# EPFL-VILAB/MultiMAE

Hardware: AMD Instinct MI355X
Metric: pre-train images/sec (whole node), ViT-B RGB+D+S 224^2 98-vis-tok (higher is better)
Workload: dtype bf16 (fp32_output_adapters: fp16 storage); 1 GPU; BASELINE.json configs[2]: ViT-B, RGB+depth+semseg, 224^2, Dirichlet alpha=1.0, 98 visible tokens, 4 cross-attention decoders (dim 256, depth 2), semseg adapter (fp32_output_adapters) with fp16 STORAGE (activations / saved tensors / gradients of the adapter as IEEE half in HBM: every matmul input carries the 11-bit significand TF32 gave the reference on A100; gradients stored times a power of two f; per_gpu_batch=256, global_batch=256, parallelism=dp1

## Files before the change

### multimae_amd/csrc/losses.hip

```cpp
#include <math.h>
#include <type_traits>
#include "common.h"

namespace {

constexpr int LSPLIT = 8;

__device__ __forceinline__ void block_sum2(float& a, float& b) {
    __shared__ float ra[4], rb[4];
    a = wave_sum(a); b = wave_sum(b);
    const int w = threadIdx.x >> 6;
    if ((threadIdx.x & 63) == 0) { ra[w] = a; rb[w] = b; }
    __syncthreads();
    if (threadIdx.x == 0) { a = (ra[0] + ra[1]) + (ra[2] + ra[3]); b = (rb[0] + rb[1]) + (rb[2] + rb[3]); }
    __syncthreads();
}

__global__ void __launch_bounds__(256) pixel_loss_fwd_kernel(const float* __restrict__ pred, const float* __restrict__ target,
                                                             const long long* __restrict__ mask, int kind, int norm_pix, int C, int H,
                                                             int W, int P, float* __restrict__ stats, float* __restrict__ partial) {
    const int b = blockIdx.y, nh = H / P, nw = W / P, np = nh * nw;
    const int lane = threadIdx.x & 63, w = threadIdx.x >> 6;
    const int npix = P * P, nval = npix * C;
    float acc = 0.f;
// ... 4 lines not shown
        if (norm_pix) {
            float s = 0.f;
            for (int e = lane; e < nval; e += 64) {
                const int c = e / npix, ij = e % npix;
                s += target[(((long long)b * C + c) * H + py * P + ij / P) * W + px * P + ij % P];
            }
            mu = wave_sum(s) / (float)nval;
            float q = 0.f;
            for (int e = lane; e < nval; e += 64) {
                const int c = e / npix, ij = e % npix;
                const float d = target[(((long long)b * C + c) * H + py * P + ij / P) * W + px * P + ij % P] - mu;
                q += d * d;
            }
            const float var = wave_sum(q) / (float)(nval - 1);
            rs = 1.0f / sqrtf(var + 1e-6f);
            if (lane == 0) { stats[((long long)b * np + p) * 2] = mu; stats[((long long)b * np + p) * 2 + 1] = rs; }
        }
        float s = 0.f;
        for (int e = lane; e < nval; e += 64) {
            const int c = e / npix, ij = e % npix;
            const long long a = (((long long)b * C + c) * H + py * P + ij / P) * W + px * P + ij % P;
            const float t = (target[a] - mu) * rs;
            const float d = pred[a] - t;
            s += kind == 0 ? d * d : fabsf(d);
        }
        s = wave_sum(s);
        if (lane == 0) acc += s;
    }
    float dummy = 0.f;
    block_sum2(acc, dummy);
    if (threadIdx.x == 0) partial[(long long)b * LSPLIT + blockIdx.x] = acc / (float)C;
}

__global__ void __launch_bounds__(256) loss_finalize_kernel(const float* __restrict__ partial, const long long* __restrict__ mask, int B,
                                                            int np, int pix_per_patch, float* __restrict__ per_sample,
                                                            float* __restrict__ loss) {
    float tot = 0.f, nvalid = 0.f;
    for (int b = threadIdx.x; b < B; b += 256) {
        float s = 0.f;
        for (int i = 0; i < LSPLIT; ++i) s += partial[(long long)b * LSPLIT + i];
        int cnt = 0;
        const long long* mrow = mask + (long long)b * np;
        int p = 0;
        if ((((uintptr_t)mrow) & 15) == 0) {
            typedef __attribute__((ext_vector_type(2))) long long ll2;
            const ll2* m2 = reinterpret_cast<const ll2*>(mrow);
            const int n2 = np >> 1;
            int q = 0;
            for (; q + 4 <= n2; q += 4) {
                const ll2 a0 = m2[q], a1 = m2[q + 1], a2 = m2[q + 2], a3 = m2[q + 3];
                cnt += (a0[0] != 0) + (a0[1] != 0) + (a1[0] != 0) + (a1[1] != 0) + (a2[0] != 0) + (a2[1] != 0) + (a3[0] != 0) + (a3[1] != 0);
            }
            for (; q < n2; ++q) { const ll2 a = m2[q]; cnt += (a[0] != 0) + (a[1] != 0); }
            p = n2 * 2;
        }
        for (; p < np; ++p) cnt += mrow[p] != 0;
        const float c = (float)cnt * (float)pix_per_patch;
        per_sample[b * 2] = s; per_sample[b * 2 + 1] = c;
        if (cnt > 0) { tot += s / c; nvalid += 1.f; }
    }
    block_sum2(tot, nvalid);
    if (threadIdx.x == 0) { loss[0] = nvalid > 0.f ? tot / nvalid : 0.f; loss[1] = nvalid; }
}

__global__ void pixel_loss_bwd_kernel(const float* __restrict__ pred, const float* __restrict__ target, const long long* __restrict__ mask,
                                      int kind, int norm_pix, int C, int H, int W, int P, const float* __restrict__ stats,
                                      const float* __restrict__ per_sample, const float* __restrict__ loss, const float* __restrict__ upstream,
                                      float* __restrict__ d_pred, long long total) {
    const long long i = (long long)blockIdx.x * blockDim.x + threadIdx.x;
    if (i >= total) return;
    const int x = (int)(i % W); long long r = i / W;
    const int y = (int)(r % H); r /= H;
    const long long b = r / C;
    const int nw = W / P, np = (H / P) * nw, p = (y / P) * nw + x / P;
    float g = 0.f;
    if (mask[b * np + p] != 0) {
        float mu = 0.f, rs = 1.f;
        if (norm_pix) { mu = stats[(b * np + p) * 2]; rs = stats[(b * np + p) * 2 + 1]; }
        const float d = pred[i] - (target[i] - mu) * rs;
        const float wgt = upstream[0] / (loss[1] * per_sample[b * 2 + 1] * (float)C);
        g = wgt * (kind == 0 ? 2.f * d : (d > 0.f ? 1.f : (d < 0.f ? -1.f : 0.f)));
    }
    d_pred[i] = g;
}

__global__ void __launch_bounds__(256) ce_fwd_kernel(const float* __restrict__ logits, const long long* __restrict__ target,
                                                     const long long* __restrict__ mask, int C, int H, int W, int P, float eps,
                                                     float* __restrict__ lse, float* __restrict__ partial) {
    const int b = blockIdx.y, HW = H * W, nw = W / P, np = (H / P) * nw;
    float acc = 0.f;
    for (int px = blockIdx.x * 256 + threadIdx.x; px < HW; px += LSPLIT * 256) {
        const int y = px / W, x = px % W;
        if (mask[(long long)b * np + (y / P) * nw + x / P] == 0) continue;
        const float* l = logits + (long long)b * C * HW + px;
        float mx = l[0], s = 1.f, sx = l[0];
// ... 259 lines not shown
            float v[8];
#pragma unroll
            for (int k = 0; k < 8; ++k) { const int e = e0 + 64 * k; v[k] = e < nval ? prow[e] : -3.0e38f; }
            float gm = fmaxf(fmaxf(fmaxf(v[0], v[1]), fmaxf(v[2], v[3])), fmaxf(fmaxf(v[4], v[5]), fmaxf(v[6], v[7])));
            if (gm > mx) { s *= expf(mx - gm); mx = gm; }
#pragma unroll
            for (int k = 0; k < 8; ++k) {
                const int e = e0 + 64 * k;
                if (e < nval) {
                    s += expf(v[k] - mx);
                    sx += v[k];
                    if ((long long)(slot + (e >> 6) * nslot) == t) lt = v[k];
                }
            }
        }
        for (int o = npix; o < 64; o <<= 1) {
            const float om = __shfl_xor(mx, o, 64), os = __shfl_xor(s, o, 64);
            lt += __shfl_xor(lt, o, 64);
            sx += __shfl_xor(sx, o, 64);
            const float nm = fmaxf(mx, om);
            s = s * expf(mx - nm) + os * expf(om - nm);
            mx = nm;
        }
        const float ls = mx + logf(s);
        if (slot == 0) { lse_pat[row * npix + pix] = ls; }
        const bool tok = t >= 0 && t < C;
        float contrib = slot == 0 && tok ? (eps == 0.f ? ls - lt : (1.f - eps) * (ls - lt) + eps * (ls - sx / (float)C)) : 0.f;
        contrib = wave_sum(contrib);
        if (lane == 0) acc += contrib;
    }
    float dummy = 0.f;
    block_sum2(acc, dummy);
    if (threadIdx.x == 0) partial[(long long)b * LSPLIT + blockIdx.x] = acc;
}

template <typename DT>
__global__ void __launch_bounds__(256) ce_pat_bwd_kernel(const float* __restrict__ pat, const long long* __restrict__ target,
                                                         const long long* __restrict__ mask, int C, int H, int W, int P, float eps,
                                                         const float* __restrict__ lse_pat, const float* __restrict__ per_sample,
                                                         const float* __restrict__ loss, const float* __restrict__ upstream,
                                                         DT* __restrict__ d_pat, long long ld, long long n_rows, float* __restrict__ amax) {
    const int lane = threadIdx.x & 63;
    const long long row = (long long)blockIdx.x * 4 + (threadIdx.x >> 6);
    const int nw = W / P, np = (H / P) * nw, npix = P * P, nval = npix * C;
    const long long b = row / np;
    const int p = (int)(row % np), py = p / nw, px = p % nw;
    const int pix = lane % npix, slot = lane / npix, nslot = 64 / npix;
    float gs = 1.0f;
    if constexpr (std::is_same<DT, h16_t>::value) {
        __shared__ float wred[4];
        const int B = (int)(n_rows / np);
        float wm = 0.f;
        for (int i = threadIdx.x; i < B; i += 256) {
            const float cnt = per_sample[i * 2 + 1];
            if (cnt > 0.f) wm = fmaxf(wm, fabsf(upstream[0] / (loss[1] * cnt)));
        }
        wm = wave_max(wm);
        if (lane == 0) wred[threadIdx.x >> 6] = wm;
        __syncthreads();
        wm = fmaxf(fmaxf(wred[0], wred[1]), fmaxf(wred[2], wred[3]));
        if (blockIdx.x == 0 && threadIdx.x == 0 && amax) *amax = wm;
        gs = h16_grad_scale(&wm);
    }
    if (row >= n_rows) return;
    const bool on = mask[row] != 0;
    DT* drow = d_pat + row * ld;
    if (!on) {
        for (int e = lane; e < (int)ld; e += 64) ActT<DT>::st(drow + e, 0.f);
        return;
    }
    const float wgt = gs * upstream[0] / (loss[1] * per_sample[b * 2 + 1]);
    const float ls = lse_pat[row * npix + pix];
    const long long t = target[((long long)b * H + py * P + pix / P) * W + px * P + pix % P];
    const bool tok = t >= 0 && t < C;
    const float* prow = pat + row * nval;
    float gmax = 0.f;
    for (int e0 = lane; e0 < (int)ld; e0 += 256) {
        float v[4];
#pragma unroll
        for (int k = 0; k < 4; ++k) { const int e = e0 + 64 * k; v[k] = e < nval ? prow[e] : 0.f; }
#pragma unroll
        for (int k = 0; k < 4; ++k) {
            const int e = e0 + 64 * k;
            if (e < (int)ld) {
                const int c = slot + (e >> 6) * nslot;
                float g = 0.f;
                if (e < nval && tok) g = wgt * (expf(v[k] - ls) - (((long long)c == t ? 1.f - eps : 0.f) + eps / (float)C));
                gmax = fmaxf(gmax, fabsf(g));
                ActT<DT>::st(drow + e, g);
            }
        }
    }
    if (!std::is_same<DT, h16_t>::value && amax) note_amax(gmax, amax);
}

__global__ void __launch_bounds__(256) sumsq_stage1(const float* __restrict__ x, long long n, float* __restrict__ ws) {
    float s = 0.f, d = 0.f;
    for (long long i = ((long long)blockIdx.x * 256 + threadIdx.x) * 4; i < n; i += (long long)gridDim.x * 1024) {
        if (i + 4 <= n) { const f32x4 v = ld4(x + i); s += (v[0] * v[0] + v[1] * v[1]) + (v[2] * v[2] + v[3] * v[3]); }
        else for (long long j = i; j < n; ++j) s += x[j] * x[j];
    }
    block_sum2(s, d);
    if (threadIdx.x == 0) ws[blockIdx.x] = s;
}
// ... 126 lines not shown
    long long nb = cdiv64(d->n, 1024);
    if (nb > 8192) nb = 8192;
    const float* bc = d->state + 5;
    const float* gsc = d->state + 2;
    if (d->shadow && d->shadow_dtype == MMAE_BF16)
        hipLaunchKernelGGL((adamw_groups_kernel<uint16_t, HY, TAIL>), dim3((unsigned)nb), dim3(256), 0, st, d->p, d->g, d->m, d->v, (long long)d->n,
                           d->group_map, (int)d->n_groups, hy, d->beta1, d->beta2, d->eps, bc, gsc, (const int*)d->istate, (uint16_t*)d->shadow, n_norm, (const float*)(d->state + 7));
    else
        hipLaunchKernelGGL((adamw_groups_kernel<float, HY, TAIL>), dim3((unsigned)nb), dim3(256), 0, st, d->p, d->g, d->m, d->v, (long long)d->n,
                           d->group_map, (int)d->n_groups, hy, d->beta1, d->beta2, d->eps, bc, gsc, (const int*)d->istate, (float*)d->shadow, n_norm, (const float*)(d->state + 7));
    return mmae_check_launch("adamw_groups");
}

inline bool shadow_ok(const void* shadow, int dtype) {
    if (!shadow) return true;
    return (dtype == MMAE_F32 && (uintptr_t)shadow % 16 == 0) || (dtype == MMAE_BF16 && (uintptr_t)shadow % 8 == 0);
}
#define MMAE_SHADOW_MSG ": shadow must be MMAE_F32 (16-byte aligned) or MMAE_BF16 (8-byte aligned)"

}

extern "C" {

int mmae_masked_pixel_loss_fwd(const float* pred, const float* target, const int64_t* mask, int kind, int norm_pix, int B, int C,
                               int H, int W, int patch, float* stats, float* partial, float* per_sample, float* loss, void* stream) {
    MMAE_REQUIRE(pred && target && mask && partial && per_sample && loss, "pixel_loss_fwd: null pointer");
    MMAE_REQUIRE(!norm_pix || stats, "pixel_loss_fwd: norm_pix needs stats");
    MMAE_REQUIRE(patch > 0 && H % patch == 0 && W % patch == 0 && (kind == 0 || kind == 1), "pixel_loss_fwd: bad geometry");
    hipStream_t st = (hipStream_t)stream;
    hipLaunchKernelGGL(pixel_loss_fwd_kernel, dim3(LSPLIT, B), dim3(256), 0, st, pred, target, (const long long*)mask, kind, norm_pix, C, H,
                       W, patch, stats, partial);
    int rc = mmae_check_launch("pixel_loss_fwd");
    if (rc) return rc;
    hipLaunchKernelGGL(loss_finalize_kernel, dim3(1), dim3(256), 0, st, partial, (const long long*)mask, B, (H / patch) * (W / patch),
                       patch * patch, per_sample, loss);
    return mmae_check_launch("loss_finalize");
}

int mmae_masked_pixel_loss_bwd(const float* pred, const float* target, const int64_t* mask, int kind, int norm_pix, int B, int C,
                               int H, int W, int patch, const float* stats, const float* per_sample, const float* loss,
                               const float* upstream, float* d_pred, void* stream) {
    MMAE_REQUIRE(pred && target && mask && per_sample && loss && upstream && d_pred, "pixel_loss_bwd: null pointer");
    const long long total = (long long)B * C * H * W;
    if (W % 4 == 0 && patch % 4 == 0 && ((uintptr_t)pred % 16 == 0) && ((uintptr_t)target % 16 == 0) && ((uintptr_t)d_pred % 16 == 0))
        hipLaunchKernelGGL(pixel_loss_bwd4_kernel, dim3((unsigned)cdiv64(total / 4, 256)), dim3(256), 0, (hipStream_t)stream, pred, target,
                           (const long long*)mask, kind, norm_pix, C, H, W, patch, stats, per_sample, loss, upstream, d_pred, total / 4);
    else
    hipLaunchKernelGGL(pixel_loss_bwd_kernel, dim3((unsigned)cdiv64(total, 256)), dim3(256), 0, (hipStream_t)stream, pred, target,
                       (const long long*)mask, kind, norm_pix, C, H, W, patch, stats, per_sample, loss, upstream, d_pred, total);
    return mmae_check_launch("pixel_loss_bwd");
}

int mmae_masked_ce_fwd(const float* logits, const int64_t* target, const int64_t* mask, int B, int C, int H, int W, int patch,
                       float label_smoothing, float* lse, float* partial, float* per_sample, float* loss, void* stream) {
    MMAE_REQUIRE(logits && target && mask && lse && partial && per_sample && loss, "ce_fwd: null pointer");
    MMAE_REQUIRE(patch > 0 && H % patch == 0 && W % patch == 0, "ce_fwd: bad geometry");
    hipStream_t st = (hipStream_t)stream;
    MMAE_REQUIRE(label_smoothing >= 0.f && label_smoothing <= 1.f, "ce_fwd: label_smoothing outside [0, 1]");
    hipLaunchKernelGGL(ce_fwd_kernel, dim3(LSPLIT, B), dim3(256), 0, st, logits, (const long long*)target, (const long long*)mask, C, H, W,
                       patch, label_smoothing, lse, partial);
    int rc = mmae_check_launch("ce_fwd");
    if (rc) return rc;
    hipLaunchKernelGGL(loss_finalize_kernel, dim3(1), dim3(256), 0, st, partial, (const long long*)mask, B, (H / patch) * (W / patch),
                       patch * patch, per_sample, loss);
    return mmae_check_launch("loss_finalize");
}

int mmae_masked_ce_bwd(const float* logits, const int64_t* target, const int64_t* mask, int B, int C, int H, int W, int patch,
                       float label_smoothing, const float* lse, const float* per_sample, const float* loss, const float* upstream,
                       float* d_logits, void* stream) {
    MMAE_REQUIRE(logits && target && mask && lse && per_sample && loss && upstream && d_logits, "ce_bwd: null pointer");
    const long long total = (long long)B * C * H * W;
    if (W % 4 == 0 && patch % 4 == 0 && ((uintptr_t)logits % 16 == 0) && ((uintptr_t)lse % 16 == 0) && ((uintptr_t)d_logits % 16 == 0))
        hipLaunchKernelGGL(ce_bwd4_kernel, dim3((unsigned)cdiv64(total / 4, 256)), dim3(256), 0, (hipStream_t)stream, logits,
                           (const long long*)target, (const long long*)mask, C, H, W, patch, label_smoothing, lse, per_sample, loss, upstream, d_logits, total / 4);
    else
    hipLaunchKernelGGL(ce_bwd_kernel, dim3((unsigned)cdiv64(total, 256)), dim3(256), 0, (hipStream_t)stream, logits, (const long long*)target,
                       (const long long*)mask, C, H, W, patch, label_smoothing, lse, per_sample, loss, upstream, d_logits, total);
    return mmae_check_launch("ce_bwd");
}

int mmae_masked_pixel_loss_pat_fwd(const float* pat, const float* target, const int64_t* mask, int kind, int norm_pix, int B, int C, int H,
                                   int W, int patch, float* stats, float* partial, float* per_sample, float* loss, void* stream) {
    MMAE_REQUIRE(pat && target && mask && partial && per_sample && loss, "pixel_loss_pat_fwd: null pointer");
    MMAE_REQUIRE(!norm_pix || stats, "pixel_loss_pat_fwd: norm_pix needs stats");
    MMAE_REQUIRE(patch > 0 && H % patch == 0 && W % patch == 0 && (kind == 0 || kind == 1), "pixel_loss_pat_fwd: bad geometry");
    hipStream_t st = (hipStream_t)stream;
    hipLaunchKernelGGL(pixel_loss_pat_fwd_kernel, dim3(LSPLIT, B), dim3(256), 0, st, pat, target, (const long long*)mask, kind, norm_pix, C, H, W,
                       patch, stats, partial);
    int rc = mmae_check_launch("pixel_loss_pat_fwd");
    if (rc) return rc;
    hipLaunchKernelGGL(loss_finalize_kernel, dim3(1), dim3(256), 0, st, partial, (const long long*)mask, B, (H / patch) * (W / patch),
                       patch * patch, per_sample, loss);
    return mmae_check_launch("loss_finalize");
}

int mmae_masked_pixel_loss_pat_bwd(const float* pat, const float* target, const int64_t* mask, int kind, int norm_pix, int B, int C, int H,
                                   int W, int patch, const float* stats, const float* per_sample, const float* loss, const float* upstream,
                                   void* d_pat, int d_pat_dtype, int64_t ld_pat, float* amax, void* stream) {
    MMAE_REQUIRE(pat && target && mask && per_sample && loss && upstream && d_pat, "pixel_loss_pat_bwd: null pointer");
    MMAE_REQUIRE(patch > 0 && H % patch == 0 && W % patch == 0 && ld_pat >= (int64_t)C * patch * patch, "pixel_loss_pat_bwd: bad geometry");
    MMAE_REQUIRE(!norm_pix || stats, "pixel_loss_pat_bwd: norm_pix needs stats");
    MMAE_REQUIRE(((uintptr_t)pat % 16 == 0) && ((uintptr_t)target % 16 == 0) && ((uintptr_t)d_pat % 16 == 0), "pixel_loss_pat_bwd: unaligned");
    const long long rows = (long long)B * (H / patch) * (W / patch);
    const dim3 grid((unsigned)((rows + 3) / 4));
    if (d_pat_dtype == MMAE_BF16)
        hipLaunchKernelGGL((pixel_loss_pat_bwd_kernel<uint16_t>), grid, dim3(256), 0, (hipStream_t)stream, pat, target, (const long long*)mask, kind,
                           norm_pix, C, H, W, patch, stats, per_sample, loss, upstream, (uint16_t*)d_pat, (long long)ld_pat, rows, amax);
    else
        hipLaunchKernelGGL((pixel_loss_pat_bwd_kernel<float>), grid, dim3(256), 0, (hipStream_t)stream, pat, target, (const long long*)mask, kind,
                           norm_pix, C, H, W, patch, stats, per_sample, loss, upstream, (float*)d_pat, (long long)ld_pat, rows, amax);
    return mmae_check_launch("pixel_loss_pat_bwd");
}

int mmae_masked_ce_pat_fwd(const float* pat, const int64_t* target, const int64_t* mask, int B, int C, int H, int W, int patch,
                           float label_smoothing, float* lse_pat, float* partial, float* per_sample, float* loss, void* stream) {
    MMAE_REQUIRE(pat && target && mask && lse_pat && partial && per_sample && loss, "ce_pat_fwd: null pointer");
    MMAE_REQUIRE(patch > 0 && H % patch == 0 && W % patch == 0, "ce_pat_fwd: bad geometry");
    const int npix = patch * patch;
    if (npix > 64 || (npix & (npix - 1))) { mmae_set_error("ce_pat_fwd: patch_size^2 must be a power of two <= 64"); return MMAE_ESUPPORT; }
    hipStream_t st = (hipStream_t)stream;
    hipLaunchKernelGGL(ce_pat_fwd_kernel, dim3(LSPLIT, B), dim3(256), 0, st, pat, (const long long*)target, (const long long*)mask, C, H, W, patch,
                       label_smoothing, lse_pat, partial);
    int rc = mmae_check_launch("ce_pat_fwd");
    if (rc) return rc;
    hipLaunchKernelGGL(loss_finalize_kernel, dim3(1), dim3(256), 0, st, partial, (const long long*)mask, B, (H / patch) * (W / patch),
                       patch * patch, per_sample, loss);
    return mmae_check_launch("loss_finalize");
}

int mmae_masked_ce_pat_bwd(const float* pat, const int64_t* target, const int64_t* mask, int B, int C, int H, int W, int patch,
                           float label_smoothing, const float* lse_pat, const float* per_sample, const float* loss, const float* upstream,
                           void* d_pat, int d_pat_dtype, int64_t ld_pat, float* amax, void* stream) {
    MMAE_REQUIRE(pat && target && mask && lse_pat && per_sample && loss && upstream && d_pat, "ce_pat_bwd: null pointer");
    MMAE_REQUIRE(patch > 0 && H % patch == 0 && W % patch == 0 && ld_pat >= (int64_t)C * patch * patch, "ce_pat_bwd: bad geometry");
    const int npix = patch * patch;
    if (npix > 64 || (npix & (npix - 1))) { mmae_set_error("ce_pat_bwd: patch_size^2 must be a power of two <= 64"); return MMAE_ESUPPORT; }
    const long long rows = (long long)B * (H / patch) * (W / patch);
    const dim3 grid((unsigned)((rows + 3) / 4));
    if (d_pat_dtype == MMAE_F16) {
        MMAE_REQUIRE(amax, "ce_pat_bwd: fp16 patch rows need the amax scalar (it carries their scale)");
        hipLaunchKernelGGL((ce_pat_bwd_kernel<h16_t>), grid, dim3(256), 0, (hipStream_t)stream, pat, (const long long*)target, (const long long*)mask,
                           C, H, W, patch, label_smoothing, lse_pat, per_sample, loss, upstream, (h16_t*)d_pat, (long long)ld_pat, rows, amax);
    } else if (d_pat_dtype == MMAE_BF16)
        hipLaunchKernelGGL((ce_pat_bwd_kernel<uint16_t>), grid, dim3(256), 0, (hipStream_t)stream, pat, (const long long*)target, (const long long*)mask,
                           C, H, W, patch, label_smoothing, lse_pat, per_sample, loss, upstream, (uint16_t*)d_pat, (long long)ld_pat, rows, amax);
    else
        hipLaunchKernelGGL((ce_pat_bwd_kernel<float>), grid, dim3(256), 0, (hipStream_t)stream, pat, (const long long*)target, (const long long*)mask,
                           C, H, W, patch, label_smoothing, lse_pat, per_sample, loss, upstream, (float*)d_pat, (long long)ld_pat, rows, amax);
    return mmae_check_launch("ce_pat_bwd");
}

int mmae_loss_split(void) { return LSPLIT; }

int mmae_sumsq(const float* x, int64_t n, float* out, float* ws, void* stream) {
    MMAE_REQUIRE(x && out && ws && n > 0, "sumsq: bad argument");
    MMAE_REQUIRE((uintptr_t)x % 16 == 0, "sumsq: unaligned");
    long long nb = cdiv64(n, 1024);
    if (nb > 1024) nb = 1024;
// ... 103 lines not shown
```

### multimae_amd/csrc/rowops.hip

```cpp
#include <stdlib.h>
#include <mutex>
#include <type_traits>
#include "common.h"

namespace {

template <int NV, typename YT, bool MXQ = false, bool STATS = true>
__global__ void __launch_bounds__(256) ln_fwd_kernel(const float* __restrict__ x, const float* __restrict__ gamma,
                                                     const float* __restrict__ beta, YT* __restrict__ y,
                                                     float* __restrict__ mean, float* __restrict__ rstd,
                                                     long long R, int D, float eps, unsigned char* __restrict__ qy = nullptr,
                                                     unsigned char* __restrict__ sc = nullptr) {
    const int lane = threadIdx.x & 63;
    const long long row = (long long)blockIdx.x * 4 + (threadIdx.x >> 6);
    if (row >= R) return;
    const float* xr = x + row * D;
    f32x4 v[NV];
    float s = 0.f;
#pragma unroll
    for (int i = 0; i < NV; ++i) {
        const int c = (lane + 64 * i) * 4;
        if (c < D) { v[i] = ld4(xr + c); s += (v[i][0] + v[i][1]) + (v[i][2] + v[i][3]); }
        else { v[i] = f32x4{0.f, 0.f, 0.f, 0.f}; }
    }
// ... 5 lines not shown
        if (c < D) {
#pragma unroll
            for (int j = 0; j < 4; ++j) { const float d = v[i][j] - mu; q += d * d; }
        }
    }
    const float var = wave_sum(q) / (float)D;
    const float rs = 1.0f / sqrtf(var + eps);
    if constexpr (STATS) {
        if (lane == 0) { mean[row] = mu; rstd[row] = rs; }
    }
    YT* yr = y + row * D;
#pragma unroll
    for (int i = 0; i < NV; ++i) {
        const int c = (lane + 64 * i) * 4;
        if (c < D) {
            const f32x4 g = ld4(gamma + c), b = ld4(beta + c);
            f32x4 o;
#pragma unroll
            for (int j = 0; j < 4; ++j) o[j] = (v[i][j] - mu) * rs * g[j] + b[j];
            st4(yr + c, o);
            if (MXQ) {
                float w[4];
#pragma unroll
                for (int j = 0; j < 4; ++j) w[j] = bf16_bits_to_f32(f32_to_bf16_bits(o[j]));
                float am = fmaxf(fmaxf(fabsf(w[0]), fabsf(w[1])), fmaxf(fabsf(w[2]), fabsf(w[3])));
                am = fmaxf(am, __shfl_xor(am, 1, 64)); am = fmaxf(am, __shfl_xor(am, 2, 64)); am = fmaxf(am, __shfl_xor(am, 4, 64));
                const int e = mx_shared_exp(am);
                const float inv = mx_inv_scale(e);
                *reinterpret_cast<int*>(qy + row * D + c) = mx_cvt4_e4m3(w[0] * inv, w[1] * inv, w[2] * inv, w[3] * inv);
                if ((lane & 7) == 0) sc[mx_scale_addr(R, row, c >> 5)] = (unsigned char)e;
            }
        }
    }
}

template <int NV, typename DT, typename AT>
__global__ void __launch_bounds__(256) ln_bwd_kernel(const DT* __restrict__ dy, const float* __restrict__ x,
                                                     const float* __restrict__ gamma, const float* __restrict__ mean,
                                                     const float* __restrict__ rstd, const float* __restrict__ dx_in,
                                                     float* __restrict__ dx_out, AT* __restrict__ dx_act,
                                                     float* __restrict__ part, long long R, int D, int part_rows) {
    __shared__ float red[2][3][NV * 256];
    const int lane = threadIdx.x & 63, w = threadIdx.x >> 6;
    f32x4 g[NV], dg[NV], db[NV], dxs[NV];
#pragma unroll
    for (int i = 0; i < NV; ++i) {
        const int c = (lane + 64 * i) * 4;
        g[i] = (c < D) ? ld4(gamma + c) : f32x4{0.f, 0.f, 0.f, 0.f};
        dg[i] = f32x4{0.f, 0.f, 0.f, 0.f};
        db[i] = f32x4{0.f, 0.f, 0.f, 0.f};
        dxs[i] = f32x4{0.f, 0.f, 0.f, 0.f};
    }
    const long long step = (long long)gridDim.x * 4;
    long long row = (long long)blockIdx.x * 4 + w;
    f32x4 nd[NV], nx[NV], na[NV];
    float nmu = 0.f, nrs = 0.f;
    auto fetch = [&](long long r) {
        nmu = mean[r]; nrs = rstd[r];
#pragma unroll
        for (int i = 0; i < NV; ++i) {
            const int c = (lane + 64 * i) * 4;
            if (c < D) {
                nd[i] = ld4(dy + r * D + c);
                nx[i] = ld4(x + r * D + c);
                if (dx_in) na[i] = ld4(dx_in + r * D + c);
            }
// ... 411 lines not shown
    if (m >= M) return;
    float a = accumulate ? out[m] : 0.f;
    for (int s = 0; s < splits; ++s) a += part[(long long)s * M + m];
    out[m] = a;
}

}

int mmae_acs_reduce(const float* part, int splits, int M, float* out, int accumulate, hipStream_t st) {
    hipLaunchKernelGGL(acs_reduce_kernel, dim3((M + 255) / 256), dim3(256), 0, st, part, splits, M, out, accumulate);
    return mmae_check_launch("acs_reduce");
}

int mmae_splitk_reduce(const float* ws, float* C, int M, int N, long long ldc, int splits, int accumulate, hipStream_t st) {
    MMAE_REQUIRE((N & 3) == 0 && (ldc & 3) == 0 && ((uintptr_t)C % 16) == 0, "gemm: split_k needs N, ldc multiples of 4 and an aligned C");
    long long nb = ((long long)M * N / 4 + 255) / 256;
    if (nb > 2048) nb = 2048;
    hipLaunchKernelGGL(splitk_reduce_kernel, dim3((unsigned)nb), dim3(256), 0, st, ws, C, M, N, ldc, splits, accumulate);
    return mmae_check_launch("splitk_reduce");
}

extern "C" {

int mmae_layernorm_fwd(const float* x, const float* gamma, const float* beta, void* y, int y_dtype, float* mean,
                       float* rstd, int64_t R, int D, float eps, void* stream) {
    MMAE_REQUIRE(x && gamma && beta && y && mean && rstd, "layernorm_fwd: null pointer");
    MMAE_REQUIRE(D % 4 == 0 && D >= 4 && D <= 1024, "layernorm_fwd: D must be a multiple of 4 in [4,1024]");
    MMAE_REQUIRE(((uintptr_t)x % 16 == 0) && ((uintptr_t)gamma % 16 == 0) && ((uintptr_t)beta % 16 == 0) && ((uintptr_t)y % 8 == 0),
                 "layernorm_fwd: unaligned pointer");
    if (R <= 0) return 0;
    const int nv = (D + 255) / 256;
    dim3 grid((unsigned)cdiv64(R, 4)), block(256);
    hipStream_t st = (hipStream_t)stream;
#define LN_FWD(NV)                                                                                                        \
    if (y_dtype == MMAE_BF16) hipLaunchKernelGGL((ln_fwd_kernel<NV, uint16_t>), grid, block, 0, st, x, gamma, beta,       \
                                                  (uint16_t*)y, mean, rstd, (long long)R, D, eps);                       \
    else if (y_dtype == MMAE_F16) hipLaunchKernelGGL((ln_fwd_kernel<NV, h16_t>), grid, block, 0, st, x, gamma, beta,      \
                                                      (h16_t*)y, mean, rstd, (long long)R, D, eps);                      \
    else hipLaunchKernelGGL((ln_fwd_kernel<NV, float>), grid, block, 0, st, x, gamma, beta, (float*)y, mean, rstd,        \
                            (long long)R, D, eps);
    switch (nv) { case 1: LN_FWD(1) break; case 2: LN_FWD(2) break; case 3: LN_FWD(3) break; default: LN_FWD(4) break; }
#undef LN_FWD
    return mmae_check_launch("layernorm_fwd");
}

int mmae_layernorm_fwd_nostat(const float* x, const float* gamma, const float* beta, void* y, int y_dtype, int64_t R, int D, float eps,
                              void* stream) {
    MMAE_REQUIRE(x && gamma && beta && y, "layernorm_fwd_nostat: null pointer");
    MMAE_REQUIRE(y_dtype == MMAE_BF16 || y_dtype == MMAE_F32, "layernorm_fwd_nostat: y is bf16 or f32");
    MMAE_REQUIRE(D % 4 == 0 && D >= 4 && D <= 1024, "layernorm_fwd_nostat: D must be a multiple of 4 in [4,1024]");
    MMAE_REQUIRE(((uintptr_t)x % 16 == 0) && ((uintptr_t)gamma % 16 == 0) && ((uintptr_t)beta % 16 == 0) && ((uintptr_t)y % 8 == 0),
                 "layernorm_fwd_nostat: unaligned pointer");
    if (R <= 0) return 0;
    const int nv = (D + 255) / 256;
    dim3 grid((unsigned)cdiv64(R, 4)), block(256);
    hipStream_t st = (hipStream_t)stream;
    float* const none = nullptr;
#define LN_FWD_NS(NV)                                                                                                                          \
    if (y_dtype == MMAE_BF16) hipLaunchKernelGGL((ln_fwd_kernel<NV, uint16_t, false, false>), grid, block, 0, st, x, gamma, beta, (uint16_t*)y, \
                                                  none, none, (long long)R, D, eps);                                                            \
    else hipLaunchKernelGGL((ln_fwd_kernel<NV, float, false, false>), grid, block, 0, st, x, gamma, beta, (float*)y, none, none, (long long)R, D, eps);
    switch (nv) { case 1: LN_FWD_NS(1) break; case 2: LN_FWD_NS(2) break; case 3: LN_FWD_NS(3) break; default: LN_FWD_NS(4) break; }
#undef LN_FWD_NS
    return mmae_check_launch("layernorm_fwd_nostat");
}

int mmae_layernorm_fwd_mx(const float* x, const float* gamma, const float* beta, void* y_bf16, float* mean, float* rstd, int64_t R, int D,
                          float eps, void* q, void* scales, void* stream) {
    MMAE_REQUIRE(x && gamma && beta && y_bf16 && mean && rstd && q && scales, "layernorm_fwd_mx: null pointer");
    MMAE_REQUIRE(D % 32 == 0 && D >= 32 && D <= 1024, "layernorm_fwd_mx: D must be a multiple of 32 in [32,1024]");
    if (R <= 0) return 0;
    const int nv = (D + 255) / 256;
    dim3 grid((unsigned)cdiv64(R, 4)), block(256);
    hipStream_t st = (hipStream_t)stream;
    if (D % 256) {
        const int rc = mmae_mx_scale_clear(scales, R, D, stream);
        if (rc) return rc;
    }
#define LN_FWD_MX(NV) hipLaunchKernelGGL((ln_fwd_kernel<NV, uint16_t, true>), grid, block, 0, st, x, gamma, beta, (uint16_t*)y_bf16, mean, rstd, \
                                         (long long)R, D, eps, (unsigned char*)q, (unsigned char*)scales);
    switch (nv) { case 1: LN_FWD_MX(1) break; case 2: LN_FWD_MX(2) break; case 3: LN_FWD_MX(3) break; default: LN_FWD_MX(4) break; }
#undef LN_FWD_MX
    return mmae_check_launch("layernorm_fwd_mx");
}

int mmae_layernorm_bwd_nblk(int64_t R) { const int64_t b = cdiv64(R, 4), cap = R >= 32768 ? 2048 : 1024; return (int)(b < 1 ? 1 : (b > cap ? cap : b)); }

int mmae_layernorm_bwd(const void* dy, int dy_dtype, const float* x, const float* gamma, const float* mean,
                       const float* rstd, const float* dx_in, float* dx_out, void* dx_act, int dx_act_dtype, float* part,
                       int64_t R, int D, void* stream) {
// ... 393 lines not shown
```

### multimae_amd/csrc/tokens.hip

```cpp
#include "common.h"

namespace {

constexpr int MAX_TASKS = 8;

struct TaskTable { int off[MAX_TASKS + 1]; int T; };

__device__ __forceinline__ int task_of(const TaskTable& tt, int idx) {
    int t = 0;
#pragma unroll
    for (int i = 1; i < MAX_TASKS; ++i) if (i < tt.T && idx >= tt.off[i]) t = i;
    return t;
}

__global__ void __launch_bounds__(256) mask_sample_kernel(const long long* __restrict__ spt, const float* __restrict__ task_noise,
                                                          const float* __restrict__ all_noise, const TaskTable tt, int Ntot,
                                                          int n_keep, long long* __restrict__ mask_all,
                                                          long long* __restrict__ ids_keep, long long* __restrict__ ids_restore) {
    extern __shared__ float sm[];
    float* noise = sm;
    int* order = (int*)(sm + Ntot);
    const int b = blockIdx.x, tid = threadIdx.x;
    for (int j = tid; j < Ntot; j += 256) noise[j] = task_noise[(long long)b * Ntot + j];
    __syncthreads();
    for (int j = tid; j < Ntot; j += 256) {
        const int t = task_of(tt, j), lo = tt.off[t], hi = tt.off[t + 1];
        const float v = noise[j];
        int rank = 0;
        for (int i = lo; i < hi; ++i) { const float u = noise[i]; rank += (u < v) || (u == v && i < j); }
        order[lo + rank] = j - lo;
    }
    __syncthreads();
    for (int j = tid; j < Ntot; j += 256) {
        const int t = task_of(tt, j);
        const int pre = (order[j] < (int)spt[(long long)b * tt.T + t]) ? 0 : 1;
        noise[j] = (float)pre + all_noise[(long long)b * Ntot + j];
    }
    __syncthreads();
    for (int j = tid; j < Ntot; j += 256) {
        const float v = noise[j];
        int rank = 0;
        for (int i = 0; i < Ntot; ++i) { const float u = noise[i]; rank += (u < v) || (u == v && i < j); }
        ids_restore[(long long)b * Ntot + j] = rank;
        mask_all[(long long)b * Ntot + j] = rank < n_keep ? 0 : 1;
        if (rank < n_keep) ids_keep[(long long)b * n_keep + rank] = j;
    }
}

struct PatchSrc {
    const void* data;
    const float* emb;
    int kind, C, H, W, ph, pw, k_off, k_len, n_cls;
};
struct PatchSrcs { PatchSrc s[MAX_TASKS]; };

template <typename RT>
__global__ void __launch_bounds__(256) patch_rows_kernel(const PatchSrcs src, const TaskTable tt, const long long* __restrict__ sel,
                                                         RT* __restrict__ rows, long long n_rows, int n_sel, int Ktot) {
    const long long row = blockIdx.x;
    const int b = (int)(row / n_sel);
    const int idx = (int)sel[row];
    const int t = task_of(tt, idx);
    const PatchSrc& s = src.s[t];
    const int p = idx - tt.off[t];
    const int nw = s.W / s.pw;
    const int py = p / nw, px = p % nw;
    RT* out = rows + row * Ktot;
    for (int k = threadIdx.x; k < Ktot; k += 256) {
        float v = 0.f;
        const int kk = k - s.k_off;
        if (kk >= 0 && kk < s.k_len) {
            const int c = kk / (s.ph * s.pw), ij = kk % (s.ph * s.pw), i = ij / s.pw, j = ij % s.pw;
            const int y = py * s.ph + i, x = px * s.pw + j;
            if (s.kind == 0) v = ((const float*)s.data)[(((long long)b * s.C + c) * s.H + y) * s.W + x];
            else {
// ... 487 lines not shown
        for (int k = 0; k < 4; ++k) atomicAdd(dst + c + k, v[k]);
    }
}

__global__ void probe_tr16_kernel(const uint16_t* __restrict__ image, const uint32_t* __restrict__ addr, uint16_t* __restrict__ out) {
    __shared__ __attribute__((aligned(16))) uint16_t lds[1024];
    for (int i = threadIdx.x; i < 1024; i += 64) lds[i] = image[i];
    __syncthreads();
    const char* p = (const char*)lds + addr[threadIdx.x];
    s16x4 v = __builtin_amdgcn_ds_read_tr16_b64_v4i16((__attribute__((address_space(3))) s16x4*)p);
#pragma unroll
    for (int j = 0; j < 4; ++j) out[threadIdx.x * 4 + j] = (uint16_t)v[j];
}

int fill_tt(TaskTable& tt, const int32_t* off_host, int T) {
    if (T < 1 || T > MAX_TASKS) return -1;
    tt.T = T;
    for (int i = 0; i <= MAX_TASKS; ++i) tt.off[i] = off_host[i <= T ? i : T];
    return 0;
}

}

extern "C" {

int mmae_mask_sample(const int64_t* samples_per_task, const float* task_noise, const float* all_noise,
                     const int32_t* task_offsets_host, int T, int B, int Ntot, int n_keep, int64_t* mask_all,
                     int64_t* ids_keep, int64_t* ids_restore, void* stream) {
    MMAE_REQUIRE(samples_per_task && task_noise && all_noise && task_offsets_host && mask_all && ids_keep && ids_restore,
                 "mask_sample: null pointer");
    TaskTable tt;
    MMAE_REQUIRE(fill_tt(tt, task_offsets_host, T) == 0, "mask_sample: 1 <= T <= 8");
    MMAE_REQUIRE(B > 0 && Ntot > 0 && Ntot <= 8192 && n_keep >= 0 && n_keep <= Ntot && tt.off[T] == Ntot, "mask_sample: bad sizes");
    hipLaunchKernelGGL(mask_sample_kernel, dim3(B), dim3(256), (size_t)Ntot * 8, (hipStream_t)stream,
                       (const long long*)samples_per_task, task_noise, all_noise, tt, Ntot, n_keep, (long long*)mask_all,
                       (long long*)ids_keep, (long long*)ids_restore);
    return mmae_check_launch("mask_sample");
}

int mmae_patch_rows(const mmae_patch_src* srcs, const int32_t* task_offsets_host, int T, const int64_t* sel, void* rows,
                    int rows_dtype, int B, int n_sel, int Ktot, void* stream) {
    MMAE_REQUIRE(srcs && task_offsets_host && sel && rows && B > 0 && n_sel > 0 && Ktot > 0, "patch_rows: bad argument");
    TaskTable tt;
    MMAE_REQUIRE(fill_tt(tt, task_offsets_host, T) == 0, "patch_rows: 1 <= T <= 8");
    if (rows_dtype != MMAE_BF16 && rows_dtype != MMAE_F32) { mmae_set_error("patch_rows: bf16 / f32 rows"); return MMAE_ESUPPORT; }
    PatchSrcs ps;
    for (int t = 0; t < MAX_TASKS; ++t) {
        const mmae_patch_src& s = srcs[t < T ? t : 0];
        MMAE_REQUIRE(s.data && s.ph > 0 && s.pw > 0 && s.H % s.ph == 0 && s.W % s.pw == 0, "patch_rows: bad source");
        MMAE_REQUIRE(s.kind == 0 || s.emb, "patch_rows: semseg source needs the class embedding");
        MMAE_REQUIRE((s.H / s.ph) * (s.W / s.pw) == tt.off[(t < T ? t : 0) + 1] - tt.off[t < T ? t : 0], "patch_rows: patch count != task tokens");
        ps.s[t] = PatchSrc{s.data, s.emb, s.kind, s.C, s.H, s.W, s.ph, s.pw, s.k_off, s.C * s.ph * s.pw, s.n_cls};
    }
    const long long n_rows = (long long)B * n_sel;
    hipStream_t st = (hipStream_t)stream;
    if (rows_dtype == MMAE_BF16) hipLaunchKernelGGL((patch_rows_kernel<uint16_t>), dim3((unsigned)n_rows), dim3(256), 0, st, ps, tt, (const long long*)sel, (uint16_t*)rows, n_rows, n_sel, Ktot);
    else hipLaunchKernelGGL((patch_rows_kernel<float>), dim3((unsigned)n_rows), dim3(256), 0, st, ps, tt, (const long long*)sel, (float*)rows, n_rows, n_sel, Ktot);
    return mmae_check_launch("patch_rows");
}

int mmae_semseg_emb_bwd(const void* d_rows, int rows_dtype, int64_t ld, const int64_t* cls, const int64_t* sel, float* d_emb,
                        int B, int H, int W, int E, int ph, int pw, int n_sel, int k_off, int tok_off, int n_patches, int n_cls,
                        void* stream) {
    MMAE_REQUIRE(d_rows && cls && sel && d_emb && B > 0 && n_cls > 0 && E > 0, "semseg_emb_bwd: bad argument");
    if (rows_dtype != MMAE_BF16 && rows_dtype != MMAE_F32) { mmae_set_error("semseg_emb_bwd: bf16 / f32 rows"); return MMAE_ESUPPORT; }
    const long long n_rows = (long long)B * n_sel;
    const int grid = (int)(n_rows < 512 ? n_rows : 512);
// ... 226 lines not shown
```

Baseline: 8865 images/s.

## Parallelize loss finalize, vectorize CE backward, add persistent LayerNorm and faster mask ranking

The loss finalize kernel now runs with 1024 threads and counts mask entries one wave per sample using ballot/popcount, where before each thread walked its own row serially. The CE patch backward kernel gains a 4-wide vectorized path for loads and stores. A grid-stride LayerNorm forward kernel for D=768 bf16 prefetches the next row while the current one is computed. The mask sampling kernel uses up to 1024 threads and a vectorized stable-rank loop. All four target small serial or latency-bound kernels in each step, at the cost of more code paths with alignment-dependent branches.

New measurement: 8918 images/s (median of 6 runs). No clear change (+0.6%).

```diff
diff --git a/multimae_amd/csrc/losses.hip b/multimae_amd/csrc/losses.hip
--- a/multimae_amd/csrc/losses.hip
+++ b/multimae_amd/csrc/losses.hip
@@ -60,35 +60,75 @@
     if (threadIdx.x == 0) partial[(long long)b * LSPLIT + blockIdx.x] = acc / (float)C;
 }
 
-__global__ void __launch_bounds__(256) loss_finalize_kernel(const float* __restrict__ partial, const long long* __restrict__ mask, int B,
-                                                            int np, int pix_per_patch, float* __restrict__ per_sample,
-                                                            float* __restrict__ loss) {
+constexpr int FIN_THREADS = 1024, FIN_WAVES = FIN_THREADS / 64, FIN_UNROLL = 4;
+
+__global__ void __launch_bounds__(FIN_THREADS) loss_finalize_kernel(const float* __restrict__ partial, const long long* __restrict__ mask,
+                                                                    int B, int np, int pix_per_patch, float* __restrict__ per_sample,
+                                                                    float* __restrict__ loss) {
+    typedef __attribute__((ext_vector_type(2))) long long ll2;
+    __shared__ int cnts[256];
+    __shared__ float ra[4], rb[4];
+    const int tid = threadIdx.x, lane = tid & 63, w = tid >> 6;
+    const bool vec = (((uintptr_t)mask) & 15) == 0 && (np & 1) == 0;
+    const int n2 = np >> 1;
     float tot = 0.f, nvalid = 0.f;
-    for (int b = threadIdx.x; b < B; b += 256) {
-        float s = 0.f;
-        for (int i = 0; i < LSPLIT; ++i) s += partial[(long long)b * LSPLIT + i];
-        int cnt = 0;
-        const long long* mrow = mask + (long long)b * np;
-        int p = 0;
-        if ((((uintptr_t)mrow) & 15) == 0) {
-            typedef __attribute__((ext_vector_type(2))) long long ll2;
-            const ll2* m2 = reinterpret_cast<const ll2*>(mrow);
-            const int n2 = np >> 1;
-            int q = 0;
-            for (; q + 4 <= n2; q += 4) {
-                const ll2 a0 = m2[q], a1 = m2[q + 1], a2 = m2[q + 2], a3 = m2[q + 3];
-                cnt += (a0[0] != 0) + (a0[1] != 0) + (a1[0] != 0) + (a1[1] != 0) + (a2[0] != 0) + (a2[1] != 0) + (a3[0] != 0) + (a3[1] != 0);
-            }
-            for (; q < n2; ++q) { const ll2 a = m2[q]; cnt += (a[0] != 0) + (a[1] != 0); }
-            p = n2 * 2;
-        }
-        for (; p < np; ++p) cnt += mrow[p] != 0;
-        const float c = (float)cnt * (float)pix_per_patch;
-        per_sample[b * 2] = s; per_sample[b * 2 + 1] = c;
-        if (cnt > 0) { tot += s / c; nvalid += 1.f; }
-    }
-    block_sum2(tot, nvalid);
-    if (threadIdx.x == 0) { loss[0] = nvalid > 0.f ? tot / nvalid : 0.f; loss[1] = nvalid; }
+    for (int base = 0; base < B; base += 256) {
+        const int nb = min(256, B - base);
+        for (int i0 = w * FIN_UNROLL; i0 < nb; i0 += FIN_WAVES * FIN_UNROLL) {
+            int cnt[FIN_UNROLL];
+#pragma unroll
+            for (int u = 0; u < FIN_UNROLL; ++u) cnt[u] = 0;
+            if (vec) {
+                for (int q0 = 0; q0 < n2; q0 += 128) {
+                    const int qa = q0 + lane, qb = q0 + 64 + lane;
+                    ll2 a[FIN_UNROLL], c[FIN_UNROLL];
+#pragma unroll
+                    for (int u = 0; u < FIN_UNROLL; ++u) {
+                        const ll2* m2 = reinterpret_cast<const ll2*>(mask + (long long)(base + min(i0 + u, nb - 1)) * np);
+                        a[u] = m2[min(qa, n2 - 1)];
+                        c[u] = m2[min(qb, n2 - 1)];
+                    }
+#pragma unroll
+                    for (int u = 0; u < FIN_UNROLL; ++u)
+                        cnt[u] += __popcll(__ballot(qa < n2 && a[u][0] != 0)) + __popcll(__ballot(qa < n2 && a[u][1] != 0)) +
+                                  __popcll(__ballot(qb < n2 && c[u][0] != 0)) + __popcll(__ballot(qb < n2 && c[u][1] != 0));
+                }
+            } else {
+                for (int p0 = 0; p0 < np; p0 += 64) {
+                    const int p = p0 + lane;
+                    long long a[FIN_UNROLL];
+#pragma unroll
+                    for (int u = 0; u < FIN_UNROLL; ++u) a[u] = mask[(long long)(base + min(i0 + u, nb - 1)) * np + min(p, np - 1)];
+#pragma unroll
+                    for (int u = 0; u < FIN_UNROLL; ++u) cnt[u] += __popcll(__ballot(p < np && a[u] != 0));
+                }
+            }
+            if (lane == 0) {
+#pragma unroll
+                for (int u = 0; u < FIN_UNROLL; ++u) if (i0 + u < nb) cnts[i0 + u] = cnt[u];
+            }
+        }
+        __syncthreads();
+        if (tid < nb) {
+            const int b = base + tid;
+            float s = 0.f;
+            for (int i = 0; i < LSPLIT; ++i) s += partial[(long long)b * LSPLIT + i];
+            const int cnt = cnts[tid];
+            const float c = (float)cnt * (float)pix_per_patch;
+            per_sample[b * 2] = s; per_sample[b * 2 + 1] = c;
+            if (cnt > 0) { tot += s / c; nvalid += 1.f; }
+        }
+        __syncthreads();
+    }
+    if (w < 4) {
+        tot = wave_sum(tot); nvalid = wave_sum(nvalid);
+        if (lane == 0) { ra[w] = tot; rb[w] = nvalid; }
+    }
+    __syncthreads();
+    if (tid == 0) {
+        tot = (ra[0] + ra[1]) + (ra[2] + ra[3]); nvalid = (rb[0] + rb[1]) + (rb[2] + rb[3]);
+        loss[0] = nvalid > 0.f ? tot / nvalid : 0.f; loss[1] = nvalid;
+    }
 }
 
 __global__ void pixel_loss_bwd_kernel(const float* __restrict__ pred, const float* __restrict__ target, const long long* __restrict__ mask,
@@ -414,6 +454,15 @@
     float dummy = 0.f;
     block_sum2(acc, dummy);
     if (threadIdx.x == 0) partial[(long long)b * LSPLIT + blockIdx.x] = acc;
+}
+
+__device__ __forceinline__ void st4_elems(float* p, f32x4 v) { st4(p, v); }
+__device__ __forceinline__ void st4_elems(h16_t* p, f32x4 v) { st4(p, v); }
+__device__ __forceinline__ void st4_elems(uint16_t* p, f32x4 v) {
+    i32x2 r;
+    r[0] = (int)((uint32_t)f32_to_bf16_bits(v[0]) | ((uint32_t)f32_to_bf16_bits(v[1]) << 16));
+    r[1] = (int)((uint32_t)f32_to_bf16_bits(v[2]) | ((uint32_t)f32_to_bf16_bits(v[3]) << 16));
+    *reinterpret_cast<i32x2*>(p) = r;
 }
 
 template <typename DT>
@@ -447,11 +496,50 @@
     if (row >= n_rows) return;
     const bool on = mask[row] != 0;
     DT* drow = d_pat + row * ld;
+    const bool vec = (npix & 3) == 0 && (ld & 3) == 0 && (((uintptr_t)pat | (uintptr_t)lse_pat) & 15) == 0 &&
+                     ((uintptr_t)d_pat % (4 * sizeof(DT))) == 0;
     if (!on) {
-        for (int e = lane; e < (int)ld; e += 64) ActT<DT>::st(drow + e, 0.f);
+        if (vec) for (int e = lane * 4; e < (int)ld; e += 256) st4_elems(drow + e, f32x4{0.f, 0.f, 0.f, 0.f});
+        else for (int e = lane; e < (int)ld; e += 64) ActT<DT>::st(drow + e, 0.f);
         return;
     }
     const float wgt = gs * upstream[0] / (loss[1] * per_sample[b * 2 + 1]);
+    if (vec) {
+        const int pix4 = (lane * 4) & (npix - 1), cshift = __ffs(npix) - 1;
+        const f32x4 ls4 = ld4(lse_pat + row * npix + pix4);
+        long long t4[4];
+#pragma unroll
+        for (int j = 0; j < 4; ++j) {
+            const int pj = pix4 + j;
+            t4[j] = target[((long long)b * H + py * P + pj / P) * W + px * P + pj % P];
+        }
+        const float* prow = pat + row * nval;
+        float gmax = 0.f;
+        for (int e0 = lane * 4; e0 < (int)ld; e0 += 1024) {
+            f32x4 v[4];
+#pragma unroll
+            for (int k = 0; k < 4; ++k) { const int e = e0 + 256 * k; v[k] = e < nval ? ld4(prow + e) : f32x4{0.f, 0.f, 0.f, 0.f}; }
+#pragma unroll
+            for (int k = 0; k < 4; ++k) {
+                const int e = e0 + 256 * k;
+                if (e < (int)ld) {
+                    const int c = e >> cshift;
+                    f32x4 g4;
+#pragma unroll
+                    for (int j = 0; j < 4; ++j) {
+                        float g = 0.f;
+                        if (e < nval && t4[j] >= 0 && t4[j] < C)
+                            g = wgt * (expf(v[k][j] - ls4[j]) - (((long long)c == t4[j] ? 1.f - eps : 0.f) + eps / (float)C));
+                        gmax = fmaxf(gmax, fabsf(g));
+                        g4[j] = g;
+                    }
+                    st4_elems(drow + e, g4);
+                }
+            }
+        }
+        if (!std::is_same<DT, h16_t>::value && amax) note_amax(gmax, amax);
+        return;
+    }
     const float ls = lse_pat[row * npix + pix];
     const long long t = target[((long long)b * H + py * P + pix / P) * W + px * P + pix % P];
     const bool tok = t >= 0 && t < C;
@@ -644,7 +732,7 @@
                        W, patch, stats, partial);
     int rc = mmae_check_launch("pixel_loss_fwd");
     if (rc) return rc;
-    hipLaunchKernelGGL(loss_finalize_kernel, dim3(1), dim3(256), 0, st, partial, (const long long*)mask, B, (H / patch) * (W / patch),
+    hipLaunchKernelGGL(loss_finalize_kernel, dim3(1), dim3(FIN_THREADS), 0, st, partial, (const long long*)mask, B, (H / patch) * (W / patch),
                        patch * patch, per_sample, loss);
     return mmae_check_launch("loss_finalize");
 }
@@ -673,7 +761,7 @@
                        patch, label_smoothing, lse, partial);
     int rc = mmae_check_launch("ce_fwd");
     if (rc) return rc;
-    hipLaunchKernelGGL(loss_finalize_kernel, dim3(1), dim3(256), 0, st, partial, (const long long*)mask, B, (H / patch) * (W / patch),
+    hipLaunchKernelGGL(loss_finalize_kernel, dim3(1), dim3(FIN_THREADS), 0, st, partial, (const long long*)mask, B, (H / patch) * (W / patch),
                        patch * patch, per_sample, loss);
     return mmae_check_launch("loss_finalize");
 }
@@ -702,7 +790,7 @@
                        patch, stats, partial);
     int rc = mmae_check_launch("pixel_loss_pat_fwd");
     if (rc) return rc;
-    hipLaunchKernelGGL(loss_finalize_kernel, dim3(1), dim3(256), 0, st, partial, (const long long*)mask, B, (H / patch) * (W / patch),
+    hipLaunchKernelGGL(loss_finalize_kernel, dim3(1), dim3(FIN_THREADS), 0, st, partial, (const long long*)mask, B, (H / patch) * (W / patch),
                        patch * patch, per_sample, loss);
     return mmae_check_launch("loss_finalize");
 }
@@ -736,7 +824,7 @@
                        label_smoothing, lse_pat, partial);
     int rc = mmae_check_launch("ce_pat_fwd");
     if (rc) return rc;
-    hipLaunchKernelGGL(loss_finalize_kernel, dim3(1), dim3(256), 0, st, partial, (const long long*)mask, B, (H / patch) * (W / patch),
+    hipLaunchKernelGGL(loss_finalize_kernel, dim3(1), dim3(FIN_THREADS), 0, st, partial, (const long long*)mask, B, (H / patch) * (W / patch),
                        patch * patch, per_sample, loss);
     return mmae_check_launch("loss_finalize");
 }
diff --git a/multimae_amd/csrc/rowops.hip b/multimae_amd/csrc/rowops.hip
--- a/multimae_amd/csrc/rowops.hip
+++ b/multimae_amd/csrc/rowops.hip
@@ -61,6 +61,78 @@
             }
         }
     }
+}
+
+constexpr int LN_FWD_WALK_WG = 4;
+template <int NV, typename YT, bool STATS>
+__global__ void __launch_bounds__(256) ln_fwd_walk_kernel(const float* __restrict__ x, const float* __restrict__ gamma,
+                                                          const float* __restrict__ beta, YT* __restrict__ y,
+                                                          float* __restrict__ mean, float* __restrict__ rstd,
+                                                          long long R, int D, float eps) {
+    const int lane = threadIdx.x & 63;
+    const long long step = (long long)gridDim.x * 4;
+    long long row = (long long)blockIdx.x * 4 + (threadIdx.x >> 6);
+    if (row >= R) return;
+    f32x4 g[NV], b[NV], nx[NV];
+#pragma unroll
+    for (int i = 0; i < NV; ++i) {
+        const int c = (lane + 64 * i) * 4;
+        g[i] = (c < D) ? ld4(gamma + c) : f32x4{0.f, 0.f, 0.f, 0.f};
+        b[i] = (c < D) ? ld4(beta + c) : f32x4{0.f, 0.f, 0.f, 0.f};
+    }
+    auto fetch = [&](long long r) {
+#pragma unroll
+        for (int i = 0; i < NV; ++i) {
+            const int c = (lane + 64 * i) * 4;
+            nx[i] = (c < D) ? ld4(x + r * D + c) : f32x4{0.f, 0.f, 0.f, 0.f};
+        }
+    };
+    fetch(row);
+    while (row < R) {
+        f32x4 v[NV];
+#pragma unroll
+        for (int i = 0; i < NV; ++i) v[i] = nx[i];
+        const long long next = row + step;
+        if (next < R) fetch(next);
+        float s = 0.f;
+#pragma unroll
+        for (int i = 0; i < NV; ++i) {
+            const int c = (lane + 64 * i) * 4;
+            if (c < D) s += (v[i][0] + v[i][1]) + (v[i][2] + v[i][3]);
+        }
+        const float mu = wave_sum(s) / (float)D;
+        float q = 0.f;
+#pragma unroll
+        for (int i = 0; i < NV; ++i) {
+            const int c = (lane + 64 * i) * 4;
+            if (c < D) {
+#pragma unroll
+                for (int j = 0; j < 4; ++j) { const float d = v[i][j] - mu; q += d * d; }
+            }
+        }
+        const float var = wave_sum(q) / (float)D;
+        const float rs = 1.0f / sqrtf(var + eps);
+        if constexpr (STATS) {
+            if (lane == 0) { mean[row] = mu; rstd[row] = rs; }
+        }
+        YT* yr = y + row * D;
+#pragma unroll
+        for (int i = 0; i < NV; ++i) {
+            const int c = (lane + 64 * i) * 4;
+            if (c < D) {
+                f32x4 o;
+#pragma unroll
+                for (int j = 0; j < 4; ++j) o[j] = (v[i][j] - mu) * rs * g[i][j] + b[i][j];
+                st4(yr + c, o);
+            }
+        }
+        row = next;
+    }
+}
+
+inline unsigned ln_fwd_walk_grid(int64_t R) {
+    const int64_t full = cdiv64(R, 4), cap = (int64_t)mmae_cu_count() * LN_FWD_WALK_WG;
+    return (unsigned)(full < cap ? full : cap);
 }
 
 template <int NV, typename DT, typename AT>
@@ -538,6 +610,11 @@
     const int nv = (D + 255) / 256;
     dim3 grid((unsigned)cdiv64(R, 4)), block(256);
     hipStream_t st = (hipStream_t)stream;
+    if (nv == 3 && y_dtype == MMAE_BF16) {
+        hipLaunchKernelGGL((ln_fwd_walk_kernel<3, uint16_t, true>), dim3(ln_fwd_walk_grid(R)), block, 0, st, x, gamma, beta,
+                           (uint16_t*)y, mean, rstd, (long long)R, D, eps);
+        return mmae_check_launch("layernorm_fwd");
+    }
 #define LN_FWD(NV)                                                                                                        \
     if (y_dtype == MMAE_BF16) hipLaunchKernelGGL((ln_fwd_kernel<NV, uint16_t>), grid, block, 0, st, x, gamma, beta,       \
                                                   (uint16_t*)y, mean, rstd, (long long)R, D, eps);                       \
@@ -562,6 +639,11 @@
     dim3 grid((unsigned)cdiv64(R, 4)), block(256);
     hipStream_t st = (hipStream_t)stream;
     float* const none = nullptr;
+    if (nv == 3 && y_dtype == MMAE_BF16) {
+        hipLaunchKernelGGL((ln_fwd_walk_kernel<3, uint16_t, false>), dim3(ln_fwd_walk_grid(R)), block, 0, st, x, gamma, beta,
+                           (uint16_t*)y, none, none, (long long)R, D, eps);
+        return mmae_check_launch("layernorm_fwd_nostat");
+    }
 #define LN_FWD_NS(NV)                                                                                                                          \
     if (y_dtype == MMAE_BF16) hipLaunchKernelGGL((ln_fwd_kernel<NV, uint16_t, false, false>), grid, block, 0, st, x, gamma, beta, (uint16_t*)y, \
                                                   none, none, (long long)R, D, eps);                                                            \
diff --git a/multimae_amd/csrc/tokens.hip b/multimae_amd/csrc/tokens.hip
--- a/multimae_amd/csrc/tokens.hip
+++ b/multimae_amd/csrc/tokens.hip
@@ -13,34 +13,57 @@
     return t;
 }
 
-__global__ void __launch_bounds__(256) mask_sample_kernel(const long long* __restrict__ spt, const float* __restrict__ task_noise,
-                                                          const float* __restrict__ all_noise, const TaskTable tt, int Ntot,
-                                                          int n_keep, long long* __restrict__ mask_all,
-                                                          long long* __restrict__ ids_keep, long long* __restrict__ ids_restore) {
-    extern __shared__ float sm[];
+constexpr int MS_THREADS = 1024;
+
+__device__ __forceinline__ int stable_rank(const float* keys, int lo, int hi, float v, int j, int jw) {
+    int rank = 0, i = lo;
+    for (; i < hi && (i & 3); ++i) { const float u = keys[i]; rank += (u < v) || (u == v && i < j); }
+    const int below = min(hi, jw);
+#pragma unroll 4
+    for (; i + 4 <= below; i += 4) {
+        const f32x4 u = *reinterpret_cast<const f32x4*>(keys + i);
+#pragma unroll
+        for (int k = 0; k < 4; ++k) rank += u[k] <= v;
+    }
+    for (; i + 4 <= hi && i <= jw + 63; i += 4) {
+        const f32x4 u = *reinterpret_cast<const f32x4*>(keys + i);
+#pragma unroll
+        for (int k = 0; k < 4; ++k) rank += (u[k] < v) || (u[k] == v && i + k < j);
+    }
+#pragma unroll 4
+    for (; i + 4 <= hi; i += 4) {
+        const f32x4 u = *reinterpret_cast<const f32x4*>(keys + i);
+#pragma unroll
+        for (int k = 0; k < 4; ++k) rank += u[k] < v;
+    }
+    for (; i < hi; ++i) { const float u = keys[i]; rank += (u < v) || (u == v && i < j); }
+    return rank;
+}
+
+__global__ void __launch_bounds__(MS_THREADS) mask_sample_kernel(const long long* __restrict__ spt, const float* __restrict__ task_noise,
+                                                                 const float* __restrict__ all_noise, const TaskTable tt, int Ntot,
+                                                                 int n_keep, long long* __restrict__ mask_all,
+                                                                 long long* __restrict__ ids_keep, long long* __restrict__ ids_restore) {
+    extern __shared__ __align__(16) float sm[];
     float* noise = sm;
     int* order = (int*)(sm + Ntot);
-    const int b = blockIdx.x, tid = threadIdx.x;
-    for (int j = tid; j < Ntot; j += 256) noise[j] = task_noise[(long long)b * Ntot + j];
+    const int b = blockIdx.x, tid = threadIdx.x, nthr = blockDim.x;
+    for (int j = tid; j < Ntot; j += nthr) noise[j] = task_noise[(long long)b * Ntot + j];
     __syncthreads();
-    for (int j = tid; j < Ntot; j += 256) {
+    for (int j = tid; j < Ntot; j += nthr) {
         const int t = task_of(tt, j), lo = tt.off[t], hi = tt.off[t + 1];
-        const float v = noise[j];
-        int rank = 0;
-        for (int i = lo; i < hi; ++i) { const float u = noise[i]; rank += (u < v) || (u == v && i < j); }
+        const int rank = stable_rank(noise, lo, hi, noise[j], j, j - (tid & 63));
         order[lo + rank] = j - lo;
     }
     __syncthreads();
-    for (int j = tid; j < Ntot; j += 256) {
+    for (int j = tid; j < Ntot; j += nthr) {
         const int t = task_of(tt, j);
         const int pre = (order[j] < (int)spt[(long long)b * tt.T + t]) ? 0 : 1;
         noise[j] = (float)pre + all_noise[(long long)b * Ntot + j];
     }
     __syncthreads();
-    for (int j = tid; j < Ntot; j += 256) {
-        const float v = noise[j];
-        int rank = 0;
-        for (int i = 0; i < Ntot; ++i) { const float u = noise[i]; rank += (u < v) || (u == v && i < j); }
+    for (int j = tid; j < Ntot; j += nthr) {
+        const int rank = stable_rank(noise, 0, Ntot, noise[j], j, j - (tid & 63));
         ids_restore[(long long)b * Ntot + j] = rank;
         mask_all[(long long)b * Ntot + j] = rank < n_keep ? 0 : 1;
         if (rank < n_keep) ids_keep[(long long)b * n_keep + rank] = j;
@@ -594,7 +617,8 @@
     TaskTable tt;
     MMAE_REQUIRE(fill_tt(tt, task_offsets_host, T) == 0, "mask_sample: 1 <= T <= 8");
     MMAE_REQUIRE(B > 0 && Ntot > 0 && Ntot <= 8192 && n_keep >= 0 && n_keep <= Ntot && tt.off[T] == Ntot, "mask_sample: bad sizes");
-    hipLaunchKernelGGL(mask_sample_kernel, dim3(B), dim3(256), (size_t)Ntot * 8, (hipStream_t)stream,
+    const int threads = Ntot >= MS_THREADS ? MS_THREADS : (Ntot + 63) / 64 * 64;
+    hipLaunchKernelGGL(mask_sample_kernel, dim3(B), dim3(threads), (size_t)Ntot * 8, (hipStream_t)stream,
                        (const long long*)samples_per_task, task_noise, all_noise, tt, Ntot, n_keep, (long long*)mask_all,
                        (long long*)ids_keep, (long long*)ids_restore);
     return mmae_check_launch("mask_sample");
```
